# ViacheslavTimofeev/tpu_superresolution

Hardware: AMD Instinct MI355X
Metric: HR pixels/sec, SwinIR x4 train step, 64x64 LR, bs=32/GPU (higher is better)
Workload: dtype bf16; 1 GPU; BASELINE cfg3: SwinIR classical x4 (dim 180, 6x6 blocks, window 8) train step = fwd + L1 + bwd + clip 1.0 + AdamW, 64x64 LR patches -> 256x256 HR, random-init weights, drop_path 0.1; every step starts from the seeded weights and fresh AdamW state; batch_per_gpu=32, global_batch=32, parallelism=dp1

## Files before the change

tpu_superresolution_amd/csrc/attn_bwd_fused.hip:

```cpp
#include "kernels.h"

namespace {

constexpr int H_K = 192, H_CA = 192, H_NH = 6;
constexpr int H_SLOT = 64 * H_K * 2;
constexpr int H_TILE = 64 * 32;
constexpr int H_PT = 64 * 64;
constexpr int H_TAB = 225;
constexpr int H_PAIR = 2 * H_SLOT;
constexpr int OFF_S = 0;
constexpr int OFF_T = 2 * H_PAIR;
constexpr int OFF_TAB = OFF_T + 12 * H_TILE * 2;
constexpr int OFF_PB = OFF_TAB + 2704;
constexpr int H_LDS = OFF_PB + 10 * 32 * 4;
static_assert(6 * H_PT * 2 == H_PAIR, "P / dS tiles of a head triple fill a row slot exactly");

#ifndef SRK_ABF_ISSUE_AT
#define SRK_ABF_ISSUE_AT 1
#endif
#ifdef SRK_PROBE_ABF
__device__ unsigned long long g_abf_probe[12 * 16 * 8];
#define ABF_MARK(k) do { if (blockIdx.x == 0 && lane == 0 && t < 16) g_abf_probe[(wave * 16 + t) * 8 + (k)] = __builtin_amdgcn_s_memrealtime(); } while (0)
extern "C" int srk_debug_abf_probe(void* host) { return (int)hipMemcpyFromSymbol(host, HIP_SYMBOL(g_abf_probe), sizeof(g_abf_probe)); }
#else
#define ABF_MARK(k) do {} while (0)
#endif

struct BwdFusedParams {
  const bf16_t* xn;
  int lda;
  const bf16_t* g;
  int ldg;
  const bf16_t* Wqkv;
  const float* bqkv;
  float scale;
  const bf16_t* WprojT;
  const float* biasd;
  bf16_t* dqkv;
  float* slab;
  long long B_;
  WinGeom geom;
};

__device__ __forceinline__ int tf(int r) { return ((((r >> 2) ^ (r >> 3)) & 1) << 1) | (((r >> 3) ^ (r >> 1)) & 1); }
__device__ __forceinline__ int ps(int r) { return (((r >> 3) & 1) << 2) | (((r >> 1) & 1) << 1) | ((r >> 2) & 1); }

__device__ __forceinline__ bf16x8_t h_cat4(bf16x4_t lo, bf16x4_t hi) {
  return bf16x8_t{lo[0], lo[1], lo[2], lo[3], hi[0], hi[1], hi[2], hi[3]};
}

__device__ __forceinline__ bf16x8_t tile_tr(const bf16_t* tile, int rb0, int rb1, int dt, int r16) {
  const int q = r16 >> 2, c = 2 * dt + ((r16 & 3) >> 1), in = (r16 & 1) << 2;
  const int ra = rb0 + q, rb = rb1 + q;
  return h_cat4(lds_tr_read(tile + ra * 32 + ((c ^ tf(ra)) << 3) + in), lds_tr_read(tile + rb * 32 + ((c ^ tf(rb)) << 3) + in));
}
__device__ __forceinline__ bf16x8_t ptile_tr(const bf16_t* tile, int rb0, int rb1, int jt, int r16) {
  const int q = r16 >> 2, c = 2 * jt + ((r16 & 3) >> 1), in = (r16 & 1) << 2;
  const int ra = rb0 + q, rb = rb1 + q;
  return h_cat4(lds_tr_read(tile + ra * 64 + ((c ^ ps(ra)) << 3) + in), lds_tr_read(tile + rb * 64 + ((c ^ ps(rb)) << 3) + in));
}

__global__ __launch_bounds__(768) void qkv_attn_bwd_kernel(const BwdFusedParams p, int ngrp) {
  extern __shared__ __attribute__((aligned(16))) unsigned char smem[];
  const unsigned smem_base = (unsigned)(size_t)smem;
  const int tid = threadIdx.x, lane = tid & 63;
  const int wave = __builtin_amdgcn_readfirstlane(tid >> 6);
  const int r16 = lane & 15, g = lane >> 4;
// ... 299 lines not shown
```

tpu_superresolution_amd/csrc/attn_fused.hip:

```cpp
#include <type_traits>

#include "kernels.h"

#ifndef SRK_NT_ATTN
#define SRK_NT_ATTN 1
#endif
#ifndef SRK_NT_STORE_QKV
#define SRK_NT_STORE_QKV 1
#endif
typedef unsigned srk_u4 __attribute__((ext_vector_type(4)));

#ifdef SRK_PROBE_ATTN
__device__ unsigned long long g_attn_probe[8 * 16 * 8];
#define ATTN_MARK(k) do { if (blockIdx.x == 0 && lane == 0 && t < 16) g_attn_probe[(wave * 16 + t) * 8 + (k)] = __builtin_amdgcn_s_memrealtime(); } while (0)
extern "C" int srk_debug_attn_probe(void* host) { return (int)hipMemcpyFromSymbol(host, HIP_SYMBOL(g_attn_probe), sizeof(g_attn_probe)); }
__device__ unsigned long long g_attn_unit_probe[8 * 3 * 8];
#define UNIT_MARK(m) do { if (blockIdx.x == 0 && lane == 0 && t == 3) g_attn_unit_probe[(wave * 3 + k) * 8 + (m)] = __builtin_readcyclecounter(); } while (0)
extern "C" int srk_debug_attn_unit_probe(void* host) { return (int)hipMemcpyFromSymbol(host, HIP_SYMBOL(g_attn_unit_probe), sizeof(g_attn_unit_probe)); }
#else
#define ATTN_MARK(k) do {} while (0)
#define UNIT_MARK(m) do {} while (0)
#endif

namespace {

// ... 197 lines not shown
  const long long nwin = (p.B_ - blockIdx.x + gridDim.x - 1) / gridDim.x;
  if (nwin <= 0) return;
  float* pbias = reinterpret_cast<float*>(smem + F_OFF_PBIAS);
  for (int i = tid; i < 3 * F_CA; i += 512) pbias[i] = p.bias ? p.bias[i] : 0.f;
  float* tab = reinterpret_cast<float*>(smem + F_OFF_TAB);
  for (int i = tid; i < F_NH * F_TAB; i += 512) {
    const int h = i / F_TAB, t = i - h * F_TAB;
    const int dy = t / 15 - 7, dx = t - (t / 15) * 15 - 7;
    const int qi = (dy > 0 ? dy : 0) * 8 + (dx > 0 ? dx : 0), kj = (dy < 0 ? -dy : 0) * 8 + (dx < 0 ? -dx : 0);
    tab[i] = p.biasd[h * 4096 + qi * 64 + kj];
  }
  if (wave < 4) fused_wave<5, false>(p, smem, wave, lane, nwin);
  else if (wave < 7) fused_wave<4, false>(p, smem, wave, lane, nwin);
  else fused_wave<4, true>(p, smem, wave, lane, nwin);
}


constexpr int G_TILE = 64 * 32;
constexpr int G_OFF_TILES = F_SLOT;
constexpr int G_OFF_PBIAS = G_OFF_TILES + 6 * G_TILE * 2;
constexpr int G_OFF_TAB = G_OFF_PBIAS + 192 * 4;
constexpr int G_LDS = G_OFF_TAB + 2 * F_TAB * 4;

__device__ __forceinline__ int g_tile_off(int row, int chunk) { return row * 32 + ((chunk ^ ((row >> 2) & 3)) << 3); }

__global__ __launch_bounds__(256, 3) void qkv_attn_fwd3_kernel(const FusedParams p, int ngrp) {
  extern __shared__ __attribute__((aligned(16))) unsigned char smem[];
  const int tid = threadIdx.x, lane = tid & 63;
  const int wave = __builtin_amdgcn_readfirstlane(tid >> 6);
  const int r16 = lane & 15, g = lane >> 4;
  const int id = blockIdx.x, xcd = id & 7, slot = id >> 3;
  const int hp = slot % 3, grp = slot / 3;
  const long long first = (long long)grp * 8 + xcd, stride = (long long)ngrp * 8;
  if (first >= p.B_) return;
  const long long nwin = (p.B_ - first + stride - 1) / stride;

  bf16_t* tiles = reinterpret_cast<bf16_t*>(smem + G_OFF_TILES);
  float* pbias = reinterpret_cast<float*>(smem + G_OFF_PBIAS);
  float* tab = reinterpret_cast<float*>(smem + G_OFF_TAB);
  for (int i = tid; i < 192; i += 256) {
    const int lf = i >> 4, which = lf >> 2, hl = (lf >> 1) & 1, half = lf & 1;
    pbias[i] = p.bias ? p.bias[which * F_CA + (2 * hp + hl) * 32 + half * 16 + (i & 15)] : 0.f;
  }
  for (int i = tid; i < 2 * F_TAB; i += 256) {
    const int hl = i / F_TAB, t = i - hl * F_TAB;
    const int dy = t / 15 - 7, dx = t - (t / 15) * 15 - 7;
    const int qi = (dy > 0 ? dy : 0) * 8 + (dx > 0 ? dx : 0), kj = (dy < 0 ? -dy : 0) * 8 + (dx < 0 ? -dx : 0);
    tab[i] = p.biasd[(2 * hp + hl) * 4096 + qi * 64 + kj];
  }

  bf16x8_t wf[3][6];
#pragma unroll
  for (int j = 0; j < 3; ++j) {
    const int lf = 3 * wave + j, which = lf >> 2, hl = (lf >> 1) & 1, half = lf & 1;
    const bf16_t* wr = p.Wt + (long long)(which * F_CA + (2 * hp + hl) * 32 + half * 16 + r16) * F_K;
#pragma unroll
    for (int s = 0; s < 6; ++s) wf[j][s] = *reinterpret_cast<const bf16x8_t*>(wr + s * 32 + g * 8);
  }

  const int srow = tid >> 2, scq = tid & 3;
  const long long grow = (long long)srow * p.lda + scq * 8;
  const int lrow = srow * (F_K * 2), lc0 = (scq ^ (srow & 7)) << 4, lc1 = lc0 ^ 64;
  uint4 pre0, pre1, pre2;
#define G_PREFETCH(BW, HALF)                                                                     \
  do {                                                                                           \
    const bf16_t* base_ = p.xn + (BW) * 64 * (long long)p.lda + grow + (HALF) * 96;              \
    pre0 = *reinterpret_cast<const uint4*>(base_);                                               \
    pre1 = *reinterpret_cast<const uint4*>(base_ + 32);                                          \
    pre2 = *reinterpret_cast<const uint4*>(base_ + 64);                                          \
  } while (0)
#define G_STAGE(HALF)                                                                            \
  do {                                                                                           \
    unsigned char* d_ = smem + lrow;                                                             \
    if ((HALF) == 0) {                                                                           \
      *reinterpret_cast<uint4*>(d_ + lc0) = pre0;                                                \
      *reinterpret_cast<uint4*>(d_ + lc1) = pre1;                                                \
      *reinterpret_cast<uint4*>(d_ + 128 + lc0) = pre2;                                          \
    } else {                                                                                     \
      *reinterpret_cast<uint4*>(d_ + 128 + lc1) = pre0;                                          \
      *reinterpret_cast<uint4*>(d_ + 256 + lc0) = pre1;                                          \
      *reinterpret_cast<uint4*>(d_ + 256 + lc1) = pre2;                                          \
    }                                                                                            \
  } while (0)
  G_PREFETCH(first, 0);
  G_STAGE(0);
  G_PREFETCH(first, 1);
  G_STAGE(1);

  const int it = wave;
  const float* tabl = tab + ((2 * it + (r16 >> 3)) - (g >> 1) + 7) * 15 + ((r16 & 7) - 4 * (g & 1) + 7) - 93;

  for (long long t = 0; t < nwin; ++t) {
    const long long b_ = first + t * stride;
    srk_lds_barrier();
    const bool more = t + 1 < nwin;
    if (more) G_PREFETCH(b_ + stride, 0);
#pragma unroll 1
    for (int mq = 0; mq < 4; ++mq) {
      f32x4_t acc[3];
#pragma unroll
      for (int j = 0; j < 3; ++j) acc[j] = f32x4_t{0.f, 0.f, 0.f, 0.f};
      const int row = 16 * mq + r16;
#pragma unroll
      for (int s = 0; s < 6; ++s) {
        const bf16x8_t xf = *reinterpret_cast<const bf16x8_t*>(smem + row * (F_K * 2) + (((s * 4 + g) ^ (row & 7)) << 4));
#pragma unroll
        for (int j = 0; j < 3; ++j) acc[j] = __builtin_amdgcn_mfma_f32_16x16x32_bf16(wf[j][s], xf, acc[j], 0, 0, 0);
      }
#pragma unroll
      for (int j = 0; j < 3; ++j) {
        const int lf = 3 * wave + j, which = lf >> 2, hl = (lf >> 1) & 1, half = lf & 1;
        const float sc = which == 0 ? p.scale : 1.0f;
        const float4 bq = *reinterpret_cast<const float4*>(pbias + 16 * lf + 4 * g);
        *reinterpret_cast<uint2*>(tiles + (which * 2 + hl) * G_TILE + g_tile_off(row, 2 * half + (g >> 1)) + 4 * (g & 1)) =
            pack_bf4((acc[j][0] + bq.x) * sc, (acc[j][1] + bq.y) * sc, (acc[j][2] + bq.z) * sc, (acc[j][3] + bq.w) * sc);
      }
    }
    srk_lds_barrier();
    if (more) {
      G_STAGE(0);
      G_PREFETCH(b_ + stride, 1);
    }
    if (p.qkv) {
      const int row = tid >> 2, ch = tid & 3;
#pragma unroll
      for (int tl = 0; tl < 6; ++tl) {
        const uint4 t4 = *reinterpret_cast<const uint4*>(tiles + tl * G_TILE + g_tile_off(row, ch));
        bf16_t* dst = p.qkv + (((tl >> 1) * p.B_ + b_) * F_NH + 2 * hp + (tl & 1)) * 2048 + row * 32 + ch * 8;
        if constexpr (SRK_NT_STORE_QKV != 0)
          __builtin_nontemporal_store(srk_u4{t4.x, t4.y, t4.z, t4.w}, reinterpret_cast<srk_u4*>(dst));
        else
          *reinterpret_cast<uint4*>(dst) = t4;
      }
    }
    {
      const int w = (int)(b_ % p.geom.nW);
      const int wy = w / p.geom.nWw, wx = w - wy * p.geom.nWw;
      const bool masked = p.geom.shift > 0 && (wy == p.geom.H / 8 - 1 || wx == p.geom.nWw - 1);
#pragma unroll 1
      for (int hl = 0; hl < 2; ++hl) {
        const bf16_t* Qs = tiles + (0 + hl) * G_TILE;
        const bf16_t* Ks = tiles + (2 + hl) * G_TILE;
        const bf16_t* Vs = tiles + (4 + hl) * G_TILE;
        const bf16x8_t qf = *reinterpret_cast<const bf16x8_t*>(Qs + g_tile_off(16 * it + r16, g));
        f32x4_t s[4];
#pragma unroll
        for (int jt = 0; jt < 4; ++jt)
          s[jt] = __builtin_amdgcn_mfma_f32_16x16x32_bf16(*reinterpret_cast<const bf16x8_t*>(Ks + g_tile_off(16 * jt + r16, g)), qf,
                                                        f32x4_t{0.f, 0.f, 0.f, 0.f}, 0, 0, 0);
        {
          const float* th = tabl + hl * F_TAB;
#pragma unroll
          for (int jt = 0; jt < 4; ++jt)
            s[jt] += f32x4_t{th[93 - 30 * jt], th[92 - 30 * jt], th[91 - 30 * jt], th[90 - 30 * jt]};
        }
        if (masked) {
          const int labi = win_region_label(p.geom, w, 16 * it + r16);
#pragma unroll
          for (int jt = 0; jt < 4; ++jt)
#pragma unroll
            for (int e = 0; e < 4; ++e)
              if (win_region_label(p.geom, w, 16 * jt + 4 * g + e) != labi) s[jt][e] += -100.0f;
        }
        bf16x8_t pf[2];
        const float inv = softmax_numerators(s, pf);
        f32x4_t o[2] = {f32x4_t{0.f, 0.f, 0.f, 0.f}, f32x4_t{0.f, 0.f, 0.f, 0.f}};
        const int ll = lane & 15;
#pragma unroll
        for (int ss = 0; ss < 2; ++ss) {
#pragma unroll
          for (int dt = 0; dt < 2; ++dt) {
            const int ch = ((2 * dt + ((ll & 3) >> 1)) ^ g) << 3, in = (ll & 1) << 2;
            const bf16x8_t vf = f_cat4(lds_tr_read(Vs + (32 * ss + 4 * g + (ll >> 2)) * 32 + ch + in),
                                       lds_tr_read(Vs + (32 * ss + 16 + 4 * g + (ll >> 2)) * 32 + ch + in));
            o[dt] = __builtin_amdgcn_mfma_f32_16x16x32_bf16(vf, pf[ss], o[dt], 0, 0, 0);
          }
        }
        o[0] *= inv;
        o[1] *= inv;
        const uint2 x = pack_bf4(o[0][0], o[0][1], o[0][2], o[0][3]), y = pack_bf4(o[1][0], o[1][1], o[1][2], o[1][3]);
        const auto s0 = __builtin_amdgcn_permlane16_swap(x.x, y.x, false, false);
        const auto s1 = __builtin_amdgcn_permlane16_swap(x.y, y.y, false, false);
        *reinterpret_cast<uint4*>(p.ao + (b_ * 64 + 16 * it + r16) * F_CA + (2 * hp + hl) * 32 + (((g & 1) << 4) | ((g >> 1) << 3))) =
            make_uint4(s0[0], s1[0], s0[1], s1[1]);
      }
    }
    if (more) G_STAGE(1);
  }
}

#ifndef SRK_ATTN_FUSED_DEFAULT
#define SRK_ATTN_FUSED_DEFAULT 2
#endif
SrkOpt g_attn_fused{OPT_ATTN_FUSED, SRK_ATTN_FUSED_DEFAULT};

}

// ... 49 lines not shown
```

tpu_superresolution_amd/csrc/gemm_stream.hip:

```cpp
#include <hip/hip_runtime.h>

#include "gemm.h"
#include "gemm_rowep.h"

namespace {

constexpr int SBN = 192;
constexpr int SBNP = SBN + 4;
constexpr int NC = SBN / 64;
constexpr int LDS_BUDGET = 160 * 1024;

#ifndef SRK_NT_GEMM
#define SRK_NT_GEMM 1
#endif
#ifndef SRK_NT_STORE_U
#define SRK_NT_STORE_U 1
#endif
typedef unsigned srk_u2 __attribute__((ext_vector_type(2)));
typedef float srk_f4 __attribute__((ext_vector_type(4)));
#ifndef SRK_NT_STORE_ALL
#define SRK_NT_STORE_ALL 0
#endif
__device__ __forceinline__ void st_u2(bf16_t* ptr, uint2 v) {
  if constexpr (SRK_NT_STORE_ALL != 0) __builtin_nontemporal_store(srk_u2{v.x, v.y}, reinterpret_cast<srk_u2*>(ptr));
  else *reinterpret_cast<uint2*>(ptr) = v;
}
__device__ __forceinline__ void st_f4(float* ptr, float4 v) {
  if constexpr (SRK_NT_STORE_ALL != 0) __builtin_nontemporal_store(srk_f4{v.x, v.y, v.z, v.w}, reinterpret_cast<srk_f4*>(ptr));
  else *reinterpret_cast<float4*>(ptr) = v;
}
__device__ __forceinline__ void glds16(const void* gsrc, unsigned lds_dst) { srk_glds16<SRK_NT_GEMM != 0>(gsrc, lds_dst); }
// ... 1 lines not shown
  unsigned keep;
  asm volatile("s_mov_b32 %0, m0\n\ts_mov_b32 m0, %2\n\ts_nop 0\n\tglobal_load_lds_dword %1, off\n\ts_mov_b32 m0, %0"
               : "=&s"(keep)
               : "v"(gsrc), "s"(lds_dst)
               : "memory");
}
template <int N>
__device__ __forceinline__ void wait_vmcnt() {
  srk_wait_vmcnt<N>();
}
__device__ __forceinline__ void lds_barrier() { srk_lds_barrier(); }

template <int EP, int KC, int BM>
struct StreamCfg {
  static constexpr int K = 64 * KC;
  static constexpr int NE32 = (EP == EP_PROJ_RES || EP == EP_RES) ? 1 : (EP == EP_LNBWD ? 2 : 0);
  static constexpr int NE16 = (EP == EP_DGELU) ? 1 : 0;
  static constexpr bool AUX = (EP == EP_PROJ_RES || EP == EP_RES || EP == EP_LNBWD);
  static constexpr int A_BYTES = BM * K * 2;
  static constexpr int E32_BYTES = BM * SBN * 4;
  static constexpr int E16_BYTES = BM * SBN * 2;
  static constexpr int AUX_BYTES = AUX ? 6 * 64 * 4 : 0;
  static constexpr int SLOT = A_BYTES + NE32 * E32_BYTES + NE16 * E16_BYTES + AUX_BYTES;
  static constexpr int T_BYTES = BM * SBNP * 4;
  static constexpr int RED_BYTES = (EP == EP_LNBWD) ? 2 * SBN * 4 : 0;
  static constexpr int CPW_A = BM * (K / 8) / 4, NI_A = (CPW_A + 63) / 64;
  static constexpr int CPW_E32 = BM * (SBN / 4) / 4, NI_E32 = (CPW_E32 + 63) / 64;
  static constexpr int CPW_E16 = BM * (SBN / 8) / 4, NI_E16 = (CPW_E16 + 63) / 64;
  static constexpr int P = NI_A + NE32 * NI_E32 + NE16 * NI_E16 + (AUX ? 1 : 0);
  static constexpr int R_LDS = (LDS_BUDGET - T_BYTES - RED_BYTES) / SLOT;
  static constexpr int R_CNT = 2 + 63 / P;
  static constexpr int R0 = R_LDS < R_CNT ? R_LDS : R_CNT;
  static constexpr int R = R0 > 8 ? 8 : (R0 < 2 ? 2 : R0);
  static constexpr bool VALID = R0 >= 2;
  static constexpr int LDS = T_BYTES + RED_BYTES + R * SLOT;
  static_assert(P * (R - 2) <= 63, "vmcnt overflow");
};

template <int EP, int KC, int BM>
struct IssueState {
  using C = StreamCfg<EP, KC, BM>;
  int aoff[C::NI_A];
  int erow[C::NE32 > 0 ? C::NI_E32 : 1];
  int eoff[C::NE32 > 0 ? C::NI_E32 : 1];
  int hoff[C::NE16 > 0 ? C::NI_E16 : 1];
  float r_nW, r_nWw, r_rps, r_ohw, r_oW;
};
// ... 209 lines not shown
        }
    }
  }
  has_scale = p.rowscale != nullptr;
}

template <int EP, int KC, int BM, int NB = 4>
__device__ __forceinline__ void stream_epilogue_tile(const GemmParams& p, const float* T, const unsigned char* slot, int m0, int n0,
                                                     int wave, int lane, EpState& st) {
  using C = StreamCfg<EP, KC, BM>;
  constexpr int MF = BM / (4 * NB);
  EP_STATE_REFS(st);
  const int sub = lane >> 4, j16 = lane & 15;
  const unsigned char* e0 = slot + C::A_BYTES;
  const float* auxf = reinterpret_cast<const float*>(slot + C::A_BYTES + C::NE32 * C::E32_BYTES + C::NE16 * C::E16_BYTES);
  const int* maps = reinterpret_cast<const int*>(auxf + 4 * 64);
#pragma unroll
  for (int ps = 0; ps < MF; ++ps) {
    const int lr = ps * (4 * NB) + wave * 4 + sub;
    const int m = m0 + lr;
    float4 v[NC];
#pragma unroll
    for (int c = 0; c < NC; ++c) {
      v[c] = *reinterpret_cast<const float4*>(T + lr * SBNP + 64 * c + 4 * j16);
      v[c].x += bias[c].x; v[c].y += bias[c].y; v[c].z += bias[c].z; v[c].w += bias[c].w;
    }
    if constexpr (EP == EP_BF16) {
#pragma unroll
      for (int c = 0; c < NC; ++c)
        st_u2(p.outb + (long long)m * p.ldo + n0 + 64 * c + 4 * j16, pack_bf4(v[c].x, v[c].y, v[c].z, v[c].w));
    } else if constexpr (EP == EP_QKV) {
      const long long b_ = m >> 6;
      const int tok = m & 63;
#pragma unroll
      for (int c = 0; c < NC; ++c) {
        const int n = n0 + 64 * c + 4 * j16;
        const int which = n / p.CA, rem = n - which * p.CA;
        const int h = rem >> 5, d = rem & 31;
        const float s = which == 0 ? p.scale : 1.0f;
        bf16_t* dst = p.outb + ((((long long)which * p.B_ + b_) * p.nH + h) * 64 + tok) * 32 + d;
        *reinterpret_cast<uint2*>(dst) = pack_bf4(v[c].x * s, v[c].y * s, v[c].z * s, v[c].w * s);
      }
    } else if constexpr (EP == EP_GELU) {
#pragma unroll
      for (int c = 0; c < NC; ++c) {
        const long long o = (long long)m * p.ldo + n0 + 64 * c + 4 * j16;
        const uint2 pu = pack_bf4(v[c].x, v[c].y, v[c].z, v[c].w);
// ... 133 lines not shown
          stream_issue_tile<EP, KC, BM>(p, is, (gi + (t + R - 1) * Gm) * BM, n0, smem_base + SLOTS_OFF + ((t + R - 1) % R) * C::SLOT, lw, lane, smem, smem_base);
      }
      if constexpr (KS2) {
        const unsigned char* As = smem + SLOTS_OFF + (t % R) * C::SLOT;
        f32x4_t acc[MF][3];
#pragma unroll
        for (int i = 0; i < MF; ++i)
#pragma unroll
          for (int j = 0; j < 3; ++j) acc[i][j] = f32x4_t{0.f, 0.f, 0.f, 0.f};
#pragma unroll
        for (int s = 0; s < KST; ++s)
#pragma unroll
          for (int i = 0; i < MF; ++i) {
            const int row = 16 * i + r16;
            const bf16x8_t xf = *reinterpret_cast<const bf16x8_t*>(As + row * (K * 2) + ((((KST + s) * 4 + g) ^ (row & 7)) << 4));
#pragma unroll
            for (int j = 0; j < 3; ++j) acc[i][j] = __builtin_amdgcn_mfma_f32_16x16x32_bf16(wf[j][s], xf, acc[i][j], 0, 0, 0);
          }
        lds_barrier();
#pragma unroll
        for (int i = 0; i < MF; ++i)
#pragma unroll
          for (int j = 0; j < 3; ++j) {
            float4* tp = reinterpret_cast<float4*>(T + (16 * i + r16) * SBNP + wn * 48 + 16 * j + 4 * g);
            float4 o = *tp;
            o.x += acc[i][j][0]; o.y += acc[i][j][1]; o.z += acc[i][j][2]; o.w += acc[i][j][3];
            *tp = o;
          }
      }
      lds_barrier();
      if constexpr (KS2) {
        if (t + R - 1 < nt)
          stream_issue_tile<EP, KC, BM>(p, is, (gi + (t + R - 1) * Gm) * BM, n0, smem_base + SLOTS_OFF + ((t + R - 1) % R) * C::SLOT, lw, lane, smem, smem_base);
      }
    }
  } else {
    EpState st;
    ep_init<EP>(p, n0, r16, st);

    for (int t = 0; t < nt; ++t) {
      const int m0 = (gi + t * Gm) * BM;
      const unsigned char* slot = smem + SLOTS_OFF + (t % R) * C::SLOT;
      lds_barrier();
      {
        f32x4_t acc[MF][3];
#pragma unroll
        for (int i = 0; i < MF; ++i)
#pragma unroll
          for (int j = 0; j < 3; ++j) acc[i][j] = f32x4_t{0.f, 0.f, 0.f, 0.f};
#pragma unroll
        for (int s = 0; s < KST; ++s)
#pragma unroll
          for (int i = 0; i < MF; ++i) {
            const int row = 16 * i + r16;
            const bf16x8_t xf = *reinterpret_cast<const bf16x8_t*>(slot + row * (K * 2) + (((s * 4 + g) ^ (row & 7)) << 4));
#pragma unroll
            for (int j = 0; j < 3; ++j) acc[i][j] = __builtin_amdgcn_mfma_f32_16x16x32_bf16(wf[j][s], xf, acc[i][j], 0, 0, 0);
          }
#pragma unroll
        for (int i = 0; i < MF; ++i)
#pragma unroll
          for (int j = 0; j < 3; ++j)
            *reinterpret_cast<float4*>(T + (16 * i + r16) * SBNP + wn * 48 + 16 * j + 4 * g) =
                make_float4(acc[i][j][0], acc[i][j][1], acc[i][j][2], acc[i][j][3]);
      }
      if constexpr (KS2) lds_barrier();
      lds_barrier();

      stream_epilogue_tile<EP, KC, BM>(p, T, slot, m0, n0, wave, lane, st);
    }
    if constexpr (EP == EP_LNBWD) {
#pragma unroll
      for (int c = 0; c < NC; ++c)
#pragma unroll
        for (int e = 0; e < 4; ++e) {
          atomicAdd(&colred[64 * c + 4 * r16 + e], st.cg[c][e]);
          atomicAdd(&colred[SBN + 64 * c + 4 * r16 + e], st.cb[c][e]);
        }
    }
  }
  if constexpr (EP == EP_LNBWD) {
    lds_barrier();
    for (int n = tid; n < p.ln_C; n += 512) {
      atomicAdd(p.ln_dgamma + n, colred[n]);
      atomicAdd(p.ln_dbeta + n, colred[SBN + n]);
    }
// ... 60 lines not shown
      if (i + R - 2 < nt)
        stream_issue_tile<EP, KC, BM>(p, is, (gi + (i + R - 2) * Gm) * BM, n0, smem_base + SLOTS_OFF + ((i + R - 2) % R) * C::SLOT, lw, lane, smem,
                                      smem_base);
      const unsigned char* slot = smem + SLOTS_OFF + (i % R) * C::SLOT;
      float* T = reinterpret_cast<float*>(smem + (i & 1) * C::T_BYTES);
      f32x4_t acc[MF][3];
#pragma unroll
      for (int a = 0; a < MF; ++a)
#pragma unroll
        for (int j = 0; j < 3; ++j) acc[a][j] = f32x4_t{0.f, 0.f, 0.f, 0.f};
#pragma unroll
      for (int s = 0; s < KST; ++s)
#pragma unroll
        for (int a = 0; a < MF; ++a) {
          const int row = 16 * a + r16;
          const bf16x8_t xf = *reinterpret_cast<const bf16x8_t*>(slot + row * (K * 2) + (((s * 4 + g) ^ (row & 7)) << 4));
#pragma unroll
          for (int j = 0; j < 3; ++j) acc[a][j] = __builtin_amdgcn_mfma_f32_16x16x32_bf16(wf[j][s], xf, acc[a][j], 0, 0, 0);
        }
#pragma unroll
      for (int a = 0; a < MF; ++a)
#pragma unroll
        for (int j = 0; j < 3; ++j)
          *reinterpret_cast<float4*>(T + (16 * a + r16) * SBNP + wn * 48 + 16 * j + 4 * g) =
              make_float4(acc[a][j][0], acc[a][j][1], acc[a][j][2], acc[a][j][3]);
    }
    lds_barrier();
  } else {
    EpState st;
    ep_init<EP>(p, n0, r16, st);
    for (int i = 0; i <= nt; ++i) {
      lds_barrier();
      if (i > 0) {
        const int t = i - 1;
        stream_epilogue_tile<EP, KC, BM, NB>(p, reinterpret_cast<const float*>(smem + (t & 1) * C::T_BYTES),
                                         smem + SLOTS_OFF + (t % R) * C::SLOT, (gi + t * Gm) * BM, n0, wave, lane, st);
      }
    }
    if constexpr (EP == EP_LNBWD) {
#pragma unroll
      for (int c = 0; c < NC; ++c)
#pragma unroll
        for (int e = 0; e < 4; ++e) {
          atomicAdd(&colred[64 * c + 4 * r16 + e], st.cg[c][e]);
          atomicAdd(&colred[SBN + 64 * c + 4 * r16 + e], st.cb[c][e]);
        }
    }
// ... 80 lines not shown
      }
      lds_barrier();
      if (i < nt) {
        if (i + R - 3 < nt)
          stream_issue_tile<EP_RES, 3, BM>(p, is, (gi + (i + R - 3) * Gm) * BM, 0, smem_base + M::SLOTS_OFF + ((i + R - 3) % R) * C::SLOT, lw,
                                           lane, smem, smem_base);
        const unsigned char* slot = smem + M::SLOTS_OFF + (i % R) * C::SLOT;
        f32x4_t acc[6];
#pragma unroll
        for (int j = 0; j < 6; ++j) acc[j] = f32x4_t{0.f, 0.f, 0.f, 0.f};
#pragma unroll
        for (int s = 0; s < 6; ++s) {
          const bf16x8_t xf = *reinterpret_cast<const bf16x8_t*>(slot + r16 * (M::K1 * 2) + (((s * 4 + g) ^ (r16 & 7)) << 4));
#pragma unroll
          for (int j = 0; j < 6; ++j) acc[j] = __builtin_amdgcn_mfma_f32_16x16x32_bf16(wf[j][s], xf, acc[j], 0, 0, 0);
        }
        unsigned char* us = Us + (i & 1) * M::UH_BYTES;
        unsigned char* hs = Hs + (i & 1) * M::UH_BYTES;
#pragma unroll
        for (int j = 0; j < 6; ++j) {
          const float4 bv = b1[j];
          const float v0 = acc[j][0] + bv.x, v1 = acc[j][1] + bv.y, v2 = acc[j][2] + bv.z, v3 = acc[j][3] + bv.w;
          const int n = lw * 96 + 16 * j + 4 * g;
          const int off = r16 * (M::HP * 2) + ((((n >> 3) ^ (r16 & 7)) << 4) | ((n & 4) << 1));
          if constexpr (DG) {
            float g0, g1, g2, g3, d0, d1, d2, d3;
            gelu_both(v0, g0, d0); gelu_both(v1, g1, d1); gelu_both(v2, g2, d2); gelu_both(v3, g3, d3);
            *reinterpret_cast<uint2*>(us + off) = pack_bf4(d0, d1, d2, d3);
            *reinterpret_cast<uint2*>(hs + off) = pack_bf4(g0, g1, g2, g3);
          } else {
            *reinterpret_cast<uint2*>(us + off) = pack_bf4(v0, v1, v2, v3);
            *reinterpret_cast<uint2*>(hs + off) = gelu_pack4(v0, v1, v2, v3);
          }
        }
      }
      lds_barrier();
    }
  } else {
    const int wn = wave;
    bf16x8_t w2[3][12];
#pragma unroll
    for (int j = 0; j < 3; ++j)
#pragma unroll
      for (int s = 0; s < 12; ++s)
        w2[j][s] = *reinterpret_cast<const bf16x8_t*>(p.W2 + (long long)(wn * 48 + 16 * j + r16) * M::HP + s * 32 + g * 8);
    const int btid = tid;
    const int sub = lane >> 4, j16 = lane & 15, lr = wave * 4 + sub;
    const bool has_scale = p.rowscale != nullptr;
    for (int i = 0; i < nt + 2; ++i) {
      lds_barrier();
      if (i >= 2) {
        const int t = i - 2;
        const unsigned char* slot = smem + M::SLOTS_OFF + (t % R) * C::SLOT;
        const unsigned char* e0 = slot + C::A_BYTES;
        const float* auxf = reinterpret_cast<const float*>(slot + C::A_BYTES + C::E32_BYTES);
        const int* maps = reinterpret_cast<const int*>(auxf + 4 * 64);
        const long long t_ = maps[lr];
        const float f = has_scale ? auxf[lr] : 1.0f;
        float4 o[NC];
#pragma unroll
        for (int c = 0; c < NC; ++c) {
          const float4 v = *reinterpret_cast<const float4*>(T2 + lr * SBNP + 64 * c + 4 * j16);
          const float4 bv = *reinterpret_cast<const float4*>(b1s + 64 * c + 4 * j16);
          const float4 rv = *reinterpret_cast<const float4*>(e0 + lr * (SBN * 4) + (64 * c + 4 * j16) * 4);
          o[c] = make_float4(rv.x + (v.x + bv.x) * f, rv.y + (v.y + bv.y) * f, rv.z + (v.z + bv.z) * f, rv.w + (v.w + bv.w) * f);
          st_f4(p.outf + t_ * p.ldo + 64 * c + 4 * j16, o[c]);
          if (p.outb) st_u2(p.outb + t_ * p.ldo + 64 * c + 4 * j16, pack_bf4(o[c].x, o[c].y, o[c].z, o[c].w));
        }
        if (p.xn_out) {
          float lg[NC][4], lb[NC][4];
#pragma unroll
          for (int c = 0; c < NC; ++c) {
            const float4 gv = *reinterpret_cast<const float4*>(b1s + SBN + 64 * c + 4 * j16);
            const float4 bb = *reinterpret_cast<const float4*>(b1s + 2 * SBN + 64 * c + 4 * j16);
            lg[c][0] = gv.x; lg[c][1] = gv.y; lg[c][2] = gv.z; lg[c][3] = gv.w;
            lb[c][0] = bb.x; lb[c][1] = bb.y; lb[c][2] = bb.z; lb[c][3] = bb.w;
          }
          fused_ln_row_at<NC>(p, o, maps[64 + lr], j16, lg, lb);
        }
      }
      f32x4_t acc[3];
      const bool have = i >= 1 && i - 1 < nt;
      if (have) {
        const unsigned char* us = Us + ((i - 1) & 1) * M::UH_BYTES;
        const unsigned char* hs = Hs + ((i - 1) & 1) * M::UH_BYTES;
#pragma unroll
        for (int j = 0; j < 3; ++j) acc[j] = f32x4_t{0.f, 0.f, 0.f, 0.f};
#pragma unroll
        for (int s = 0; s < 12; ++s) {
          const bf16x8_t xf = *reinterpret_cast<const bf16x8_t*>(hs + r16 * (M::HP * 2) + (((s * 4 + g) ^ (r16 & 7)) << 4));
#pragma unroll
          for (int j = 0; j < 3; ++j) acc[j] = __builtin_amdgcn_mfma_f32_16x16x32_bf16(w2[j][s], xf, acc[j], 0, 0, 0);
        }
        if (p.u_out) {
          const long long m0 = (long long)(gi + (i - 1) * Gm) * BM;
          int bt = btid;
          asm volatile("" : "+v"(bt));
#pragma unroll 1
          for (int it = 0; it < 3; ++it) {
            const int idx = it * 256 + bt;
            const int row = idx / 48, c = idx - row * 48;
            const int off = row * (M::HP * 2) + ((c ^ (row & 7)) << 4);
            const uint4 uv = *reinterpret_cast<const uint4*>(us + off);
            const uint4 hv = *reinterpret_cast<const uint4*>(hs + off);
            typedef unsigned srk_u4 __attribute__((ext_vector_type(4)));
            __builtin_nontemporal_store(srk_u4{uv.x, uv.y, uv.z, uv.w}, reinterpret_cast<srk_u4*>(p.u_out + (m0 + row) * p.HP + c * 8));
            __builtin_nontemporal_store(srk_u4{hv.x, hv.y, hv.z, hv.w}, reinterpret_cast<srk_u4*>(p.h_out + (m0 + row) * p.HP + c * 8));
          }
        }
      }
      lds_barrier();
      if (have) {
#pragma unroll
        for (int j = 0; j < 3; ++j)
          *reinterpret_cast<float4*>(T2 + r16 * SBNP + wn * 48 + 16 * j + 4 * g) = make_float4(acc[j][0], acc[j][1], acc[j][2], acc[j][3]);
      }
    }
  }
}

struct MlpBwdCfg {
  using CB = StreamCfg<EP_LNBWD, 0, 16>;
  static constexpr int BM = 16, K1 = 192, HP = 384, RF = 3, RB = 2;
  static constexpr int A_BYTES = BM * K1 * 2;
  static constexpr int U_BYTES = BM * HP * 2;
  static constexpr int FSLOT = A_BYTES + U_BYTES;
  static constexpr int PF = 2 + 3;
  static constexpr int PB = CB::P;
  static constexpr int T2_OFF = 0;
  static constexpr int RED_OFF = CB::T_BYTES;
  static constexpr int GAM_OFF = RED_OFF + 4 * 2 * SBN * 4;
  static constexpr int DS_OFF = GAM_OFF + SBN * 4;
  static constexpr int FS_OFF = DS_OFF + 2 * U_BYTES;
  static constexpr int BS_OFF = FS_OFF + RF * FSLOT;
  static constexpr int LDS = BS_OFF + RB * CB::SLOT;
  static_assert(CB::A_BYTES == 0 && CB::NI_A == 0, "back slot carries no A image");
  static_assert(LDS <= LDS_BUDGET, "fused MLP backward: LDS budget");
  static_assert(PF + PB <= 63, "vmcnt overflow");
// ... 28 lines not shown
    const int lw = wave - 4;
    bf16x8_t wf[6][6];
#pragma unroll
    for (int j = 0; j < 6; ++j)
#pragma unroll
      for (int s = 0; s < 6; ++s)
        wf[j][s] = *reinterpret_cast<const bf16x8_t*>(p.Wt + (long long)(lw * 96 + 16 * j + r16) * M::K1 + s * 32 + g * 8);
#pragma unroll
    for (int j = 0; j < 6; ++j)
#pragma unroll
      for (int s = 0; s < 6; ++s) asm volatile("" ::"v"(wf[j][s]));

    int aoff[2], uoff[3];
#pragma unroll
    for (int i = 0; i < 2; ++i) {
      const int qq = lw * 96 + i * 64 + lane;
      const int row = qq / 24, pos = qq - row * 24;
      aoff[i] = row * p.lda + ((pos ^ (row & 7)) << 3);
    }
#pragma unroll
    for (int i = 0; i < 3; ++i) {
      const int qq = lw * 192 + i * 64 + lane;
      const int row = qq / 48, pos = qq - row * 48;
      uoff[i] = row * p.HP + ((pos ^ (row & 7)) << 3);
    }
    auto issue_front = [&](int t) {
      const long long m0 = (long long)(gi + t * Gm) * BM;
      const unsigned slot = smem_base + M::FS_OFF + (t % M::RF) * M::FSLOT;
      const bf16_t* ab = p.A + m0 * p.lda;
      const bf16_t* ub = p.aux + m0 * p.HP;
      glds16(ab + aoff[0], __builtin_amdgcn_readfirstlane(slot + (lw * 96) * 16));
      if (lane < 32) glds16(ab + aoff[1], __builtin_amdgcn_readfirstlane(slot + (lw * 96 + 64) * 16));
#pragma unroll
      for (int i = 0; i < 3; ++i) glds16(ub + uoff[i], __builtin_amdgcn_readfirstlane(slot + M::A_BYTES + (lw * 192 + i * 64) * 16));
    };
    IssueState<EP_LNBWD, 0, BM> is;
    issue_init<EP_LNBWD, 0, BM>(p, 0, lw, lane, is);
    auto issue_back = [&](int t) {
      stream_issue_tile<EP_LNBWD, 0, BM>(p, is, (gi + t * Gm) * BM, 0, smem_base + M::BS_OFF + (t % M::RB) * CB::SLOT, lw, lane, smem, smem_base);
    };

    for (int s = 0; s < M::RF - 1 && s < nt; ++s) issue_front(s);
    for (int i = 0; i < nt + 2; ++i) {
      if (i + 1 < nt && i >= 1) wait_vmcnt<M::PF + M::PB>();
      else if (i + 1 < nt) wait_vmcnt<M::PF>();
      else wait_vmcnt<0>();
      lds_barrier();
      if (i < nt) {
        if (i + M::RF - 1 < nt) issue_front(i + M::RF - 1);
        const unsigned char* slot = smem + M::FS_OFF + (i % M::RF) * M::FSLOT;
        const unsigned char* uimg = slot + M::A_BYTES;
        f32x4_t acc[6];
#pragma unroll
        for (int j = 0; j < 6; ++j) acc[j] = f32x4_t{0.f, 0.f, 0.f, 0.f};
#pragma unroll
        for (int s = 0; s < 6; ++s) {
          const bf16x8_t xf = *reinterpret_cast<const bf16x8_t*>(slot + r16 * (M::K1 * 2) + (((s * 4 + g) ^ (r16 & 7)) << 4));
#pragma unroll
          for (int j = 0; j < 6; ++j) acc[j] = __builtin_amdgcn_mfma_f32_16x16x32_bf16(wf[j][s], xf, acc[j], 0, 0, 0);
        }
        unsigned char* ds = Ds + (i & 1) * M::U_BYTES;
#pragma unroll
        for (int j = 0; j < 6; ++j) {
          const int n = lw * 96 + 16 * j + 4 * g;
          const int off = r16 * (M::HP * 2) + ((((n >> 3) ^ (r16 & 7)) << 4) | ((n & 4) << 1));
          const uint2 ua = *reinterpret_cast<const uint2*>(uimg + off);
          float u0, u1, u2, u3;
          unpack_bf2(ua.x, u0, u1);
          unpack_bf2(ua.y, u2, u3);
          if constexpr (DG) *reinterpret_cast<uint2*>(ds + off) = pack_bf4(acc[j][0] * u0, acc[j][1] * u1, acc[j][2] * u2, acc[j][3] * u3);
          else *reinterpret_cast<uint2*>(ds + off) = dgelu_mul_pack4(acc[j][0], acc[j][1], acc[j][2], acc[j][3], u0, u1, u2, u3);
        }
      }
      lds_barrier();
      if (i < nt) issue_back(i);
    }
  } else {
    const int wn = wave;
    bf16x8_t w2[3][12];
#pragma unroll
    for (int j = 0; j < 3; ++j)
#pragma unroll
      for (int s = 0; s < 12; ++s)
        w2[j][s] = *reinterpret_cast<const bf16x8_t*>(p.W2 + (long long)(wn * 48 + 16 * j + r16) * M::HP + s * 32 + g * 8);
    const int btid = tid;
    const int sub = lane >> 4, j16 = lane & 15, lr = wave * 4 + sub;
    const float invC = 1.0f / (float)p.ln_C;
    const bool has_scale = p.rowscale != nullptr;
    for (int i = 0; i < nt + 2; ++i) {
      lds_barrier();
      if (i >= 2) {
        const int t = i - 2;
        const unsigned char* slot = smem + M::BS_OFF + (t % M::RB) * CB::SLOT;
        const float* auxf = reinterpret_cast<const float*>(slot + 2 * CB::E32_BYTES);
        const int* maps = reinterpret_cast<const int*>(auxf + 4 * 64);
        const long long t_ = maps[lr], ro = maps[64 + lr];
        const float mean = auxf[lr], rstd = auxf[64 + lr];
        const float f = has_scale ? auxf[128 + lr] : 1.0f;
        float dy[NC][4], xh[NC][4];
        float s1 = 0.f, s2 = 0.f;
#pragma unroll
        for (int c = 0; c < NC; ++c) {
          const float4 dv = *reinterpret_cast<const float4*>(T2 + lr * SBNP + 64 * c + 4 * j16);
          const float4 xv = *reinterpret_cast<const float4*>(slot + lr * (SBN * 4) + (64 * c + 4 * j16) * 4);
          const float4 gv = *reinterpret_cast<const float4*>(gam + 64 * c + 4 * j16);
          const float dvs[4] = {dv.x, dv.y, dv.z, dv.w}, xs[4] = {xv.x, xv.y, xv.z, xv.w}, gs[4] = {gv.x, gv.y, gv.z, gv.w};
#pragma unroll
          for (int e = 0; e < 4; ++e) {
            dy[c][e] = dvs[e];
            xh[c][e] = 64 * c + 4 * j16 + e < p.ln_C ? (xs[e] - mean) * rstd : 0.f;
            const float dg = dvs[e] * gs[e];
            s1 += dg;
            s2 += dg * xh[c][e];
          }
        }
        s1 = wave_sum16(s1) * invC;
        s2 = wave_sum16(s2) * invC;
        float* myred = colred + wave * (2 * SBN);
#pragma unroll
        for (int c = 0; c < NC; ++c) {
          const float4 old = *reinterpret_cast<const float4*>(slot + CB::E32_BYTES + lr * (SBN * 4) + (64 * c + 4 * j16) * 4);
          const float4 gv = *reinterpret_cast<const float4*>(gam + 64 * c + 4 * j16);
          const float gs[4] = {gv.x, gv.y, gv.z, gv.w};
          float o[4] = {old.x, old.y, old.z, old.w};
          float pg[4], pb[4];
#pragma unroll
// ... 2 lines not shown
            o[e] += live ? rstd * (dy[c][e] * gs[e] - s1 - xh[c][e] * s2) : 0.f;
            pg[e] = xrow_sum4(dy[c][e] * xh[c][e]);
            pb[e] = xrow_sum4(live ? dy[c][e] : 0.f);
          }
          if (sub == 0) {
            float4* rg = reinterpret_cast<float4*>(myred + 64 * c + 4 * j16);
            float4* rb = reinterpret_cast<float4*>(myred + SBN + 64 * c + 4 * j16);
            const float4 a = *rg, b = *rb;
            *rg = make_float4(a.x + pg[0], a.y + pg[1], a.z + pg[2], a.w + pg[3]);
            *rb = make_float4(b.x + pb[0], b.y + pb[1], b.z + pb[2], b.w + pb[3]);
          }
          st_f4(p.outf + t_ * p.ldo + 64 * c + 4 * j16, make_float4(o[0], o[1], o[2], o[3]));
          if (p.outb) st_u2(p.outb + ro * p.ldo + 64 * c + 4 * j16, pack_bf4(o[0] * f, o[1] * f, o[2] * f, o[3] * f));
        }
      }
      f32x4_t acc[3];
      const bool have = i >= 1 && i - 1 < nt;
      if (have) {
        const unsigned char* ds = Ds + ((i - 1) & 1) * M::U_BYTES;
#pragma unroll
        for (int j = 0; j < 3; ++j) acc[j] = f32x4_t{0.f, 0.f, 0.f, 0.f};
#pragma unroll
        for (int s = 0; s < 12; ++s) {
          const bf16x8_t xf = *reinterpret_cast<const bf16x8_t*>(ds + r16 * (M::HP * 2) + (((s * 4 + g) ^ (r16 & 7)) << 4));
#pragma unroll
          for (int j = 0; j < 3; ++j) acc[j] = __builtin_amdgcn_mfma_f32_16x16x32_bf16(w2[j][s], xf, acc[j], 0, 0, 0);
        }
        {
          const long long m0 = (long long)(gi + (i - 1) * Gm) * BM;
          int bt = btid;
          asm volatile("" : "+v"(bt));
#pragma unroll 1
          for (int it = 0; it < 3; ++it) {
            const int idx = it * 256 + bt;
            const int row = idx / 48, c = idx - row * 48;
            const uint4 dv = *reinterpret_cast<const uint4*>(ds + row * (M::HP * 2) + ((c ^ (row & 7)) << 4));
            *reinterpret_cast<uint4*>(p.u_out + (m0 + row) * p.HP + c * 8) = dv;
          }
        }
      }
      lds_barrier();
      if (have) {
#pragma unroll
        for (int j = 0; j < 3; ++j)
          *reinterpret_cast<float4*>(T2 + r16 * SBNP + wn * 48 + 16 * j + 4 * g) = make_float4(acc[j][0], acc[j][1], acc[j][2], acc[j][3]);
      }
    }
  }
  lds_barrier();
  for (int n = tid; n < p.ln_C; n += 512) {
    atomicAdd(p.ln_dgamma + n, (colred[n] + colred[2 * SBN + n]) + (colred[4 * SBN + n] + colred[6 * SBN + n]));
    atomicAdd(p.ln_dbeta + n, (colred[SBN + n] + colred[3 * SBN + n]) + (colred[5 * SBN + n] + colred[7 * SBN + n]));
  }
}

SrkOpt g_mlp_fused_enabled{OPT_MLP_FUSED, 1};
SrkOpt g_mlp_bwd_fused_enabled{OPT_MLP_BWD_FUSED, 1};
SrkOpt g_mlp_dgelu_store{OPT_MLP_DGELU_STORE, 1};

SrkOpt g_stream_enabled{OPT_GEMM_STREAM, -1};
thread_local int g_num_cus = 0;
SrkOpt g_tune_bm{OPT_TUNE_BM, 0};
SrkOpt g_tune_ks2{OPT_TUNE_KS2, -1};
SrkOpt g_tune_split{OPT_TUNE_SPLIT, -1};
SrkOpt g_tune_nb{OPT_TUNE_NB, 0};

template <typename KernelT>
int stream_configure(KernelT kernel, int lds, int* state) {
// ... 213 lines not shown
```

Before: 73.31 million HR pixels/s.

## Centralize LDS swizzle layouts and change swizzles to cut bank conflicts

```diff
diff --git a/tpu_superresolution_amd/csrc/attn_bwd_fused.hip b/tpu_superresolution_amd/csrc/attn_bwd_fused.hip
--- a/tpu_superresolution_amd/csrc/attn_bwd_fused.hip
+++ b/tpu_superresolution_amd/csrc/attn_bwd_fused.hip
@@ -1,4 +1,5 @@
 #include "kernels.h"
+#include "lds_layout.h"
 
 namespace {
 
@@ -42,7 +43,7 @@
   WinGeom geom;
 };
 
-__device__ __forceinline__ int tf(int r) { return ((((r >> 2) ^ (r >> 3)) & 1) << 1) | (((r >> 3) ^ (r >> 1)) & 1); }
+__device__ __forceinline__ int tf(int r) { return srk_lds::head_swz(r); }
 __device__ __forceinline__ int ps(int r) { return (((r >> 3) & 1) << 2) | (((r >> 1) & 1) << 1) | ((r >> 2) & 1); }
 
 __device__ __forceinline__ bf16x8_t h_cat4(bf16x4_t lo, bf16x4_t hi) {
diff --git a/tpu_superresolution_amd/csrc/attn_fused.hip b/tpu_superresolution_amd/csrc/attn_fused.hip
--- a/tpu_superresolution_amd/csrc/attn_fused.hip
+++ b/tpu_superresolution_amd/csrc/attn_fused.hip
@@ -1,6 +1,7 @@
 #include <type_traits>
 
 #include "kernels.h"
+#include "lds_layout.h"
 
 #ifndef SRK_NT_ATTN
 #define SRK_NT_ATTN 1
@@ -244,8 +245,6 @@
 constexpr int G_OFF_TAB = G_OFF_PBIAS + 192 * 4;
 constexpr int G_LDS = G_OFF_TAB + 2 * F_TAB * 4;
 
-__device__ __forceinline__ int g_tile_off(int row, int chunk) { return row * 32 + ((chunk ^ ((row >> 2) & 3)) << 3); }
-
 __global__ __launch_bounds__(256, 3) void qkv_attn_fwd3_kernel(const FusedParams p, int ngrp) {
   extern __shared__ __attribute__((aligned(16))) unsigned char smem[];
   const int tid = threadIdx.x, lane = tid & 63;
@@ -282,7 +281,7 @@
 
   const int srow = tid >> 2, scq = tid & 3;
   const long long grow = (long long)srow * p.lda + scq * 8;
-  const int lrow = srow * (F_K * 2), lc0 = (scq ^ (srow & 7)) << 4, lc1 = lc0 ^ 64;
+  const int lrow = srow * (F_K * 2), lc0 = srk_lds::xrow_off(srow, scq) - lrow, lc1 = srk_lds::xrow_off(srow, scq + 4) - lrow;
   uint4 pre0, pre1, pre2;
 #define G_PREFETCH(BW, HALF)                                                                     \
   do {                                                                                           \
@@ -325,7 +324,7 @@
       const int row = 16 * mq + r16;
 #pragma unroll
       for (int s = 0; s < 6; ++s) {
-        const bf16x8_t xf = *reinterpret_cast<const bf16x8_t*>(smem + row * (F_K * 2) + (((s * 4 + g) ^ (row & 7)) << 4));
+        const bf16x8_t xf = *reinterpret_cast<const bf16x8_t*>(smem + srk_lds::xrow_off(row, s * 4 + g));
 #pragma unroll
         for (int j = 0; j < 3; ++j) acc[j] = __builtin_amdgcn_mfma_f32_16x16x32_bf16(wf[j][s], xf, acc[j], 0, 0, 0);
       }
@@ -334,7 +333,7 @@
         const int lf = 3 * wave + j, which = lf >> 2, hl = (lf >> 1) & 1, half = lf & 1;
         const float sc = which == 0 ? p.scale : 1.0f;
         const float4 bq = *reinterpret_cast<const float4*>(pbias + 16 * lf + 4 * g);
-        *reinterpret_cast<uint2*>(tiles + (which * 2 + hl) * G_TILE + g_tile_off(row, 2 * half + (g >> 1)) + 4 * (g & 1)) =
+        *reinterpret_cast<uint2*>(tiles + (which * 2 + hl) * G_TILE + srk_lds::head_off(row, 2 * half + (g >> 1)) + 4 * (g & 1)) =
             pack_bf4((acc[j][0] + bq.x) * sc, (acc[j][1] + bq.y) * sc, (acc[j][2] + bq.z) * sc, (acc[j][3] + bq.w) * sc);
       }
     }
@@ -347,7 +346,7 @@
       const int row = tid >> 2, ch = tid & 3;
 #pragma unroll
       for (int tl = 0; tl < 6; ++tl) {
-        const uint4 t4 = *reinterpret_cast<const uint4*>(tiles + tl * G_TILE + g_tile_off(row, ch));
+        const uint4 t4 = *reinterpret_cast<const uint4*>(tiles + tl * G_TILE + srk_lds::head_off(row, ch));
         bf16_t* dst = p.qkv + (((tl >> 1) * p.B_ + b_) * F_NH + 2 * hp + (tl & 1)) * 2048 + row * 32 + ch * 8;
         if constexpr (SRK_NT_STORE_QKV != 0)
           __builtin_nontemporal_store(srk_u4{t4.x, t4.y, t4.z, t4.w}, reinterpret_cast<srk_u4*>(dst));
@@ -364,11 +363,11 @@
         const bf16_t* Qs = tiles + (0 + hl) * G_TILE;
         const bf16_t* Ks = tiles + (2 + hl) * G_TILE;
         const bf16_t* Vs = tiles + (4 + hl) * G_TILE;
-        const bf16x8_t qf = *reinterpret_cast<const bf16x8_t*>(Qs + g_tile_off(16 * it + r16, g));
+        const bf16x8_t qf = *reinterpret_cast<const bf16x8_t*>(Qs + srk_lds::head_off(16 * it + r16, g));
         f32x4_t s[4];
 #pragma unroll
         for (int jt = 0; jt < 4; ++jt)
-          s[jt] = __builtin_amdgcn_mfma_f32_16x16x32_bf16(*reinterpret_cast<const bf16x8_t*>(Ks + g_tile_off(16 * jt + r16, g)), qf,
+          s[jt] = __builtin_amdgcn_mfma_f32_16x16x32_bf16(*reinterpret_cast<const bf16x8_t*>(Ks + srk_lds::head_off(16 * jt + r16, g)), qf,
                                                         f32x4_t{0.f, 0.f, 0.f, 0.f}, 0, 0, 0);
         {
           const float* th = tabl + hl * F_TAB;
@@ -392,9 +391,9 @@
         for (int ss = 0; ss < 2; ++ss) {
 #pragma unroll
           for (int dt = 0; dt < 2; ++dt) {
-            const int ch = ((2 * dt + ((ll & 3) >> 1)) ^ g) << 3, in = (ll & 1) << 2;
-            const bf16x8_t vf = f_cat4(lds_tr_read(Vs + (32 * ss + 4 * g + (ll >> 2)) * 32 + ch + in),
-                                       lds_tr_read(Vs + (32 * ss + 16 + 4 * g + (ll >> 2)) * 32 + ch + in));
+            const int ch = 2 * dt + ((ll & 3) >> 1), in = (ll & 1) << 2;
+            const bf16x8_t vf = f_cat4(lds_tr_read(Vs + srk_lds::head_off(32 * ss + 4 * g + (ll >> 2), ch) + in),
+                                       lds_tr_read(Vs + srk_lds::head_off(32 * ss + 16 + 4 * g + (ll >> 2), ch) + in));
             o[dt] = __builtin_amdgcn_mfma_f32_16x16x32_bf16(vf, pf[ss], o[dt], 0, 0, 0);
           }
         }
diff --git a/tpu_superresolution_amd/csrc/gemm_stream.hip b/tpu_superresolution_amd/csrc/gemm_stream.hip
--- a/tpu_superresolution_amd/csrc/gemm_stream.hip
+++ b/tpu_superresolution_amd/csrc/gemm_stream.hip
@@ -2,11 +2,11 @@
 
 #include "gemm.h"
 #include "gemm_rowep.h"
+#include "lds_layout.h"
 
 namespace {
 
 constexpr int SBN = 192;
-constexpr int SBNP = SBN + 4;
 constexpr int NC = SBN / 64;
 constexpr int LDS_BUDGET = 160 * 1024;
 
@@ -54,7 +54,7 @@
   static constexpr int E16_BYTES = BM * SBN * 2;
   static constexpr int AUX_BYTES = AUX ? 6 * 64 * 4 : 0;
   static constexpr int SLOT = A_BYTES + NE32 * E32_BYTES + NE16 * E16_BYTES + AUX_BYTES;
-  static constexpr int T_BYTES = BM * SBNP * 4;
+  static constexpr int T_BYTES = BM * srk_lds::ACC_PITCH * 4;
   static constexpr int RED_BYTES = (EP == EP_LNBWD) ? 2 * SBN * 4 : 0;
   static constexpr int CPW_A = BM * (K / 8) / 4, NI_A = (CPW_A + 63) / 64;
   static constexpr int CPW_E32 = BM * (SBN / 4) / 4, NI_E32 = (CPW_E32 + 63) / 64;
@@ -310,7 +310,7 @@
     float4 v[NC];
 #pragma unroll
     for (int c = 0; c < NC; ++c) {
-      v[c] = *reinterpret_cast<const float4*>(T + lr * SBNP + 64 * c + 4 * j16);
+      v[c] = *reinterpret_cast<const float4*>(T + srk_lds::acc_off(lr, 64 * c + 4 * j16));
       v[c].x += bias[c].x; v[c].y += bias[c].y; v[c].z += bias[c].z; v[c].w += bias[c].w;
     }
     if constexpr (EP == EP_BF16) {
@@ -490,7 +490,7 @@
         for (int i = 0; i < MF; ++i)
 #pragma unroll
           for (int j = 0; j < 3; ++j) {
-            float4* tp = reinterpret_cast<float4*>(T + (16 * i + r16) * SBNP + wn * 48 + 16 * j + 4 * g);
+            float4* tp = reinterpret_cast<float4*>(T + srk_lds::acc_off(16 * i + r16, wn * 48 + 16 * j + 4 * g));
             float4 o = *tp;
             o.x += acc[i][j][0]; o.y += acc[i][j][1]; o.z += acc[i][j][2]; o.w += acc[i][j][3];
             *tp = o;
@@ -529,7 +529,7 @@
         for (int i = 0; i < MF; ++i)
 #pragma unroll
           for (int j = 0; j < 3; ++j)
-            *reinterpret_cast<float4*>(T + (16 * i + r16) * SBNP + wn * 48 + 16 * j + 4 * g) =
+            *reinterpret_cast<float4*>(T + srk_lds::acc_off(16 * i + r16, wn * 48 + 16 * j + 4 * g)) =
                 make_float4(acc[i][j][0], acc[i][j][1], acc[i][j][2], acc[i][j][3]);
       }
       if constexpr (KS2) lds_barrier();
@@ -636,7 +636,7 @@
       for (int a = 0; a < MF; ++a)
 #pragma unroll
         for (int j = 0; j < 3; ++j)
-          *reinterpret_cast<float4*>(T + (16 * a + r16) * SBNP + wn * 48 + 16 * j + 4 * g) =
+          *reinterpret_cast<float4*>(T + srk_lds::acc_off(16 * a + r16, wn * 48 + 16 * j + 4 * g)) =
               make_float4(acc[a][j][0], acc[a][j][1], acc[a][j][2], acc[a][j][3]);
     }
     lds_barrier();
@@ -763,7 +763,7 @@
           const float4 bv = b1[j];
           const float v0 = acc[j][0] + bv.x, v1 = acc[j][1] + bv.y, v2 = acc[j][2] + bv.z, v3 = acc[j][3] + bv.w;
           const int n = lw * 96 + 16 * j + 4 * g;
-          const int off = r16 * (M::HP * 2) + ((((n >> 3) ^ (r16 & 7)) << 4) | ((n & 4) << 1));
+          const int off = srk_lds::hid_off(r16, n >> 3) + ((n & 4) << 1);
           if constexpr (DG) {
             float g0, g1, g2, g3, d0, d1, d2, d3;
             gelu_both(v0, g0, d0); gelu_both(v1, g1, d1); gelu_both(v2, g2, d2); gelu_both(v3, g3, d3);
@@ -801,7 +801,7 @@
         float4 o[NC];
 #pragma unroll
         for (int c = 0; c < NC; ++c) {
-          const float4 v = *reinterpret_cast<const float4*>(T2 + lr * SBNP + 64 * c + 4 * j16);
+          const float4 v = *reinterpret_cast<const float4*>(T2 + srk_lds::acc_off(lr, 64 * c + 4 * j16));
           const float4 bv = *reinterpret_cast<const float4*>(b1s + 64 * c + 4 * j16);
           const float4 rv = *reinterpret_cast<const float4*>(e0 + lr * (SBN * 4) + (64 * c + 4 * j16) * 4);
           o[c] = make_float4(rv.x + (v.x + bv.x) * f, rv.y + (v.y + bv.y) * f, rv.z + (v.z + bv.z) * f, rv.w + (v.w + bv.w) * f);
@@ -829,7 +829,7 @@
         for (int j = 0; j < 3; ++j) acc[j] = f32x4_t{0.f, 0.f, 0.f, 0.f};
 #pragma unroll
         for (int s = 0; s < 12; ++s) {
-          const bf16x8_t xf = *reinterpret_cast<const bf16x8_t*>(hs + r16 * (M::HP * 2) + (((s * 4 + g) ^ (r16 & 7)) << 4));
+          const bf16x8_t xf = *reinterpret_cast<const bf16x8_t*>(hs + srk_lds::hid_off(r16, s * 4 + g));
 #pragma unroll
           for (int j = 0; j < 3; ++j) acc[j] = __builtin_amdgcn_mfma_f32_16x16x32_bf16(w2[j][s], xf, acc[j], 0, 0, 0);
         }
@@ -841,7 +841,7 @@
           for (int it = 0; it < 3; ++it) {
             const int idx = it * 256 + bt;
             const int row = idx / 48, c = idx - row * 48;
-            const int off = row * (M::HP * 2) + ((c ^ (row & 7)) << 4);
+            const int off = srk_lds::hid_off(row, c);
             const uint4 uv = *reinterpret_cast<const uint4*>(us + off);
             const uint4 hv = *reinterpret_cast<const uint4*>(hs + off);
             typedef unsigned srk_u4 __attribute__((ext_vector_type(4)));
@@ -854,7 +854,7 @@
       if (have) {
 #pragma unroll
         for (int j = 0; j < 3; ++j)
-          *reinterpret_cast<float4*>(T2 + r16 * SBNP + wn * 48 + 16 * j + 4 * g) = make_float4(acc[j][0], acc[j][1], acc[j][2], acc[j][3]);
+          *reinterpret_cast<float4*>(T2 + srk_lds::acc_off(r16, wn * 48 + 16 * j + 4 * g)) = make_float4(acc[j][0], acc[j][1], acc[j][2], acc[j][3]);
       }
     }
   }
@@ -929,7 +929,7 @@
     for (int i = 0; i < 3; ++i) {
       const int qq = lw * 192 + i * 64 + lane;
       const int row = qq / 48, pos = qq - row * 48;
-      uoff[i] = row * p.HP + ((pos ^ (row & 7)) << 3);
+      uoff[i] = row * p.HP + (srk_lds::hid_chunk(row, pos) << 3);
     }
     auto issue_front = [&](int t) {
       const long long m0 = (long long)(gi + t * Gm) * BM;
@@ -970,7 +970,7 @@
 #pragma unroll
         for (int j = 0; j < 6; ++j) {
           const int n = lw * 96 + 16 * j + 4 * g;
-          const int off = r16 * (M::HP * 2) + ((((n >> 3) ^ (r16 & 7)) << 4) | ((n & 4) << 1));
+          const int off = srk_lds::hid_off(r16, n >> 3) + ((n & 4) << 1);
           const uint2 ua = *reinterpret_cast<const uint2*>(uimg + off);
           float u0, u1, u2, u3;
           unpack_bf2(ua.x, u0, u1);
@@ -1008,7 +1008,7 @@
         float s1 = 0.f, s2 = 0.f;
 #pragma unroll
         for (int c = 0; c < NC; ++c) {
-          const float4 dv = *reinterpret_cast<const float4*>(T2 + lr * SBNP + 64 * c + 4 * j16);
+          const float4 dv = *reinterpret_cast<const float4*>(T2 + srk_lds::acc_off(lr, 64 * c + 4 * j16));
           const float4 xv = *reinterpret_cast<const float4*>(slot + lr * (SBN * 4) + (64 * c + 4 * j16) * 4);
           const float4 gv = *reinterpret_cast<const float4*>(gam + 64 * c + 4 * j16);
           const float dvs[4] = {dv.x, dv.y, dv.z, dv.w}, xs[4] = {xv.x, xv.y, xv.z, xv.w}, gs[4] = {gv.x, gv.y, gv.z, gv.w};
@@ -1057,7 +1057,7 @@
         for (int j = 0; j < 3; ++j) acc[j] = f32x4_t{0.f, 0.f, 0.f, 0.f};
 #pragma unroll
         for (int s = 0; s < 12; ++s) {
-          const bf16x8_t xf = *reinterpret_cast<const bf16x8_t*>(ds + r16 * (M::HP * 2) + (((s * 4 + g) ^ (r16 & 7)) << 4));
+          const bf16x8_t xf = *reinterpret_cast<const bf16x8_t*>(ds + srk_lds::hid_off(r16, s * 4 + g));
 #pragma unroll
           for (int j = 0; j < 3; ++j) acc[j] = __builtin_amdgcn_mfma_f32_16x16x32_bf16(w2[j][s], xf, acc[j], 0, 0, 0);
         }
@@ -1069,7 +1069,7 @@
           for (int it = 0; it < 3; ++it) {
             const int idx = it * 256 + bt;
             const int row = idx / 48, c = idx - row * 48;
-            const uint4 dv = *reinterpret_cast<const uint4*>(ds + row * (M::HP * 2) + ((c ^ (row & 7)) << 4));
+            const uint4 dv = *reinterpret_cast<const uint4*>(ds + srk_lds::hid_off(row, c));
             *reinterpret_cast<uint4*>(p.u_out + (m0 + row) * p.HP + c * 8) = dv;
           }
         }
@@ -1078,7 +1078,7 @@
       if (have) {
 #pragma unroll
         for (int j = 0; j < 3; ++j)
-          *reinterpret_cast<float4*>(T2 + r16 * SBNP + wn * 48 + 16 * j + 4 * g) = make_float4(acc[j][0], acc[j][1], acc[j][2], acc[j][3]);
+          *reinterpret_cast<float4*>(T2 + srk_lds::acc_off(r16, wn * 48 + 16 * j + 4 * g)) = make_float4(acc[j][0], acc[j][1], acc[j][2], acc[j][3]);
       }
     }
   }
diff --git a/tpu_superresolution_amd/csrc/lds_layout.h b/tpu_superresolution_amd/csrc/lds_layout.h
--- /dev/null
+++ b/tpu_superresolution_amd/csrc/lds_layout.h
@@ -0,0 +1,31 @@
+#pragma once
+
+#if defined(__HIP__) || defined(__HIPCC__)
+#define SRK_LDS_FN __host__ __device__ constexpr inline
+#else
+#define SRK_LDS_FN constexpr inline
+#endif
+
+namespace srk_lds {
+
+constexpr int HID_ROW_BYTES = 768;
+SRK_LDS_FN int hid_chunk(int row, int chunk) { return chunk ^ (row & 15); }
+SRK_LDS_FN int hid_off(int row, int chunk) {
+  return row * HID_ROW_BYTES + ((chunk >> 4) << 8) + (((chunk & 15) ^ (row & 15)) << 4);
+}
+
+constexpr int ACC_PITCH = 192;
+SRK_LDS_FN int acc_off(int row, int col) {
+  return row * ACC_PITCH + (col & ~63) + ((((col >> 2) & 15) ^ (row & 15)) << 2);
+}
+
+SRK_LDS_FN int head_swz(int row) { return ((((row >> 2) ^ (row >> 3)) & 1) << 1) | (((row >> 3) ^ (row >> 1)) & 1); }
+SRK_LDS_FN int head_off(int row, int chunk) {
+  return row * 32 + ((chunk ^ head_swz(row & 15)) << 3);
+}
+
+constexpr int XROW_BYTES = 384;
+SRK_LDS_FN int xrow_swz(int row) { return (row & 7) ^ ((row & 1) << 2); }
+SRK_LDS_FN int xrow_off(int row, int chunk) { return row * XROW_BYTES + ((chunk ^ xrow_swz(row)) << 4); }
+
+}
```

Result: no change. 73.95 million HR pixels/s (median of 6 runs) (+0.9%).
